# noisystreet/aither

Measured on AMD Instinct MI355X. Metric: Mcell-updates/sec per iteration (residual+LU-SGS), 256^3 block; % HBM roofline, higher is better.
Workload: dtype f64

## Files before the change

### aither_amd/csrc/agx_lusgs.hpp

```cpp
#pragma once
#include "agx_device.hpp"

namespace agx {

enum {
  PA_S = 0,
  PA_B = 3,
  PA_X = 6,
  PA_F = 9,
  PA_COUNT = 15,
  D1_VF = 2 * PA_COUNT,
  D1_AD = D1_VF + 1,
  D2_DOUBLES = 2 * PA_COUNT + 4
};

struct D2Dev {
  double* base;
  long nd2, ps;
  const int* dstart;
  const int* ij_of_pos;
  int Pi, Pj;
  __device__ __forceinline__ double2* pa(int id) const {
    return reinterpret_cast<double2*>(base + 2L * id * nd2);
  }
  __device__ __forceinline__ double* vf() const { return base + (long)D1_VF * nd2; }
  __device__ __forceinline__ double* ad(int d) const { return base + (long)(D1_AD + d) * nd2; }
  __device__ __forceinline__ double ld_ad(int d, long cell) const { return ad(d)[cell]; }
  __device__ __forceinline__ double2 ld_pair(int id, long cell) const { return pa(id)[cell]; }
  __device__ __forceinline__ double ld_vf(long cell) const { return vf()[cell]; }
  __device__ __forceinline__ int jlo(int de) const { return max(0, de - (Pi - 1)); }
  __device__ __forceinline__ int pos2(int ie, int je) const {
    const int de = ie + je;
    return dstart[de] + je - jlo(de);
  }
};

struct KpBlk {
  double* base;
  const int* dstart;
  const agx_bc_surface* surf;
  long nd2, ps;
  int Pi, Pj, ni, nj, nk, ng;
  int nsurf, nsurf_i, nsurf_j, nsurf_k;
  int side_conn[6];
  __device__ __forceinline__ int dstart_cf(int de) const {
    const int a = min(Pi, Pj), bm = max(Pi, Pj);
    if (de <= a) return de * (de + 1) / 2;
    if (de <= bm) return a * (a + 1) / 2 + (de - a) * a;
    const int r = Pi + Pj - 1 - de;
    return Pi * Pj - r * (r + 1) / 2;
  }
  __device__ __forceinline__ const char* pab(int id) const {
    return reinterpret_cast<const char*>(base) + (size_t)id * (size_t)nd2 * 16;
  }
  __device__ __forceinline__ const char* vfb() const {
    return reinterpret_cast<const char*>(base) + (size_t)D1_VF * (size_t)nd2 * 8;
  }
  __device__ __forceinline__ const char* adb(int d) const {
    return reinterpret_cast<const char*>(base) + (size_t)(D1_AD + d) * (size_t)nd2 * 8;
  }
  __device__ __forceinline__ double ld_ad(int d, long cell) const {
    return *reinterpret_cast<const double*>(adb(d) + cell * 8);
  }
  __device__ __forceinline__ double2 ld_pair(int id, long cell) const {
    return *reinterpret_cast<const double2*>(pab(id) + cell * 16);
  }
  __device__ __forceinline__ double ld_vf(long cell) const {
    return *reinterpret_cast<const double*>(vfb() + cell * 8);
  }
  __device__ __forceinline__ int jlo(int de) const { return max(0, de - (Pi - 1)); }
};
struct KpGas { double hf, n, inv_n; };
__device__ __forceinline__ double2 ld16(const char* ubase, unsigned voff) {
  return *reinterpret_cast<const double2*>(ubase + voff);
}
__device__ __forceinline__ double ld8(const char* ubase, unsigned voff) {
  return *reinterpret_cast<const double*>(ubase + voff);
}

}
```

### aither_amd/csrc/agx_lusgs_kernels.hpp

```cpp
#pragma once

namespace agx {

constexpr int TT = 32;
constexpr int TRS = TT + 2;
__device__ __forceinline__ int tile_diag_index(int li, int lj) {
  const int dd = li + lj;
  if (dd < TT) return dd * (dd + 1) / 2 + lj;
  const int r = 2 * TT - 2 - dd;
  return TT * TT - (r + 1) * (r + 2) / 2 + (lj - (dd - (TT - 1)));
}
__device__ __forceinline__ void tile_table(unsigned short* s_tab) {
  const int tid = threadIdx.x;
#pragma unroll
  for (int m = 0; m < 4; ++m) {
    const int li = tid & (TT - 1), lj = (tid >> 5) + 8 * m;
    s_tab[tile_diag_index(li, lj)] = (unsigned short)(li | (lj << 8));
  }
}

__device__ __forceinline__ double kp_tagged(double v, unsigned tag) {
  const unsigned long long u = (unsigned long long)__double_as_longlong(v);
  return __longlong_as_double((long long)((u & ~3ull) | tag));
}
__device__ __forceinline__ bool kp_has_tag(double v, unsigned tag) {
  return ((unsigned)__double_as_longlong(v) & 3u) == tag;
}
__device__ __forceinline__ double cell_visc_factor(const GasDev& g, const double* s) {
  if (!(s[0] > 0.0)) return 0.0;
  return visc_max_term(g, s[0]) * visc_term(g, viscosity(g, temperature(g, s)));
}

__global__ void __launch_bounds__(256) k_d2_geo(BlockDev b) {
  const D2Dev& z = b.d2;
  const long t = (long)blockIdx.x * blockDim.x + threadIdx.x;
  const long n = (long)z.Pi * z.Pj * (b.nk + 2 * b.ng);
  if (t >= n) return;
  const int e3[3] = {(int)(t % z.Pi), (int)((t / z.Pi) % z.Pj), (int)(t / ((long)z.Pi * z.Pj))};
  const long q = b.idx(e3[0] - b.ng, e3[1] - b.ng, e3[2] - b.ng);
  const long p = (long)e3[2] * z.ps + z.pos2(e3[0], e3[1]);
#pragma unroll
  for (int d = 0; d < 3; ++d) {
    double a[4];
#pragma unroll
    for (int c = 0; c < 4; ++c) a[c] = b.fa[d][c][q];
    double ad = 0.0;
    if (e3[d] > 0) {
      const long ql = q - b.stride(d);
      const double v[3] = {b.cen[0][q] - b.cen[0][ql], b.cen[1][q] - b.cen[1][ql],
                           b.cen[2][q] - b.cen[2][ql]};
      const double dist = dot3(v, a);
      ad = dist != 0.0 ? a[3] / dist : 0.0;
    }
    z.pa(PA_F + 2 * d + 0)[p] = make_double2(a[0], a[1]);
    z.pa(PA_F + 2 * d + 1)[p] = make_double2(a[2], a[3]);
    z.ad(d)[p] = ad;
  }
}
__global__ void __launch_bounds__(256) k_d2_x_copy(BlockDev b, int to_d2, unsigned tag) {
  const D2Dev& z = b.d2;
  const long t = (long)blockIdx.x * blockDim.x + threadIdx.x;
  const long n = (long)z.Pi * z.Pj * (b.nk + 2 * b.ng);
  if (t >= n) return;
  const int ie = (int)(t % z.Pi), je = (int)((t / z.Pi) % z.Pj),
            ke = (int)(t / ((long)z.Pi * z.Pj));
  const long q = b.idx(ie - b.ng, je - b.ng, ke - b.ng);
  const long p = (long)ke * z.ps + z.pos2(ie, je);
#pragma unroll
  for (int e = 0; e < AGX_NEQ; ++e) {
    double* xp = reinterpret_cast<double*>(z.pa(PA_X + (e >> 1))) + 2 * p + (e & 1);
    if (to_d2) *xp = kp_tagged(b.x[e][q], tag);
    else b.x[e][q] = *xp;
  }
}

__global__ void __launch_bounds__(256)
k_lusgs_prepare(BlockDev b, GasDev g, SolverDev sp, int write_x, unsigned tag, int again) {
  __shared__ double sv[6][TT][TRS];
  __shared__ unsigned short s_tab[TT * TT];
  const D2Dev& z = b.d2;
  const int tid = threadIdx.x;
  tile_table(s_tab);
  const int i0 = blockIdx.x * TT, j0 = blockIdx.y * TT, ke = blockIdx.z;
  const int k = ke - b.ng;
  const int li = tid & (TT - 1);
  double bb[4][AGX_NEQ], x0[4][AGX_NEQ], ainv[4], vf[4];
#pragma unroll
  for (int m = 0; m < 4; ++m) {
    const int lj = (tid >> 5) + 8 * m;
    const int ie = i0 + li, je = j0 + lj;
    const int i = ie - b.ng, j = je - b.ng;
#pragma unroll
    for (int e = 0; e < AGX_NEQ; ++e) { bb[m][e] = 0.0; x0[m][e] = 0.0; }
    ainv[m] = 1.0;
    vf[m] = 0.0;
    double cs = 0.0;
    if (ie < z.Pi && je < z.Pj) {
      const long q = b.idx(i, j, k);
      double s[AGX_NEQ];
#pragma unroll
      for (int e = 0; e < AGX_NEQ; ++e) { s[e] = b.state[e][q]; sv[e][lj][li] = s[e]; }
      if (s[0] > 0.0) cs = sound_speed(g, s);
      if (sp.viscous) vf[m] = cell_visc_factor(g, s);
      const bool phys = i >= 0 && i < b.ni && j >= 0 && j < b.nj && k >= 0 && k < b.nk;
      if (phys) {
        double dvt = (b.vol[q] * (1.0 + sp.zeta)) / (b.dt[q] * sp.theta);
        if (sp.dual_time_cfl > 0.0) dvt += fmax(b.specrad[q], 0.0) / sp.dual_time_cfl;
        const double a = again ? b.ainv[q] : b.a[q] * sp.relax + dvt;
        b.ainv[q] = a;
        if (sp.diag_add) b.a[q] = a;
        ainv[m] = 1.0 / a;
        rhs_bf(b, g, sp, q, bb[m]);
        if (sp.requires_init) {
#pragma unroll
          for (int e = 0; e < AGX_NEQ; ++e) x0[m][e] = bb[m][e] * ainv[m];
        }
      }
    }
    sv[5][lj][li] = cs;
  }
  __syncthreads();
  long pos[4];
  int tli[4], tlj[4];
#pragma unroll
  for (int m = 0; m < 4; ++m) {
    const unsigned tl = s_tab[tid + 256 * m];
    tli[m] = tl & 0xff; tlj[m] = tl >> 8;
    const int ie = i0 + tli[m], je = j0 + tlj[m];
    pos[m] = -1;
    if (ie < z.Pi && je < z.Pj) {
      pos[m] = (long)ke * z.ps + z.pos2(ie, je);
#pragma unroll
      for (int h = 0; h < 3; ++h)
        z.pa(PA_S + h)[pos[m]] = make_double2(sv[2 * h][tlj[m]][tli[m]], sv[2 * h + 1][tlj[m]][tli[m]]);
    }
  }
  __syncthreads();
#pragma unroll
  for (int m = 0; m < 4; ++m) {
    const int lj = (tid >> 5) + 8 * m;
#pragma unroll
    for (int e = 0; e < AGX_NEQ; ++e) sv[e][lj][li] = bb[m][e];
    sv[5][lj][li] = ainv[m];
  }
  __syncthreads();
  double ai2[4];
#pragma unroll
  for (int m = 0; m < 4; ++m) {
    ai2[m] = sv[5][tlj[m]][tli[m]];
    if (pos[m] >= 0) {
#pragma unroll
      for (int h = 0; h < 3; ++h)
        z.pa(PA_B + h)[pos[m]] = make_double2(sv[2 * h][tlj[m]][tli[m]], sv[2 * h + 1][tlj[m]][tli[m]]);
    }
  }
  __syncthreads();
#pragma unroll
  for (int m = 0; m < 4; ++m) {
    const int lj = (tid >> 5) + 8 * m;
#pragma unroll
    for (int e = 0; e < AGX_NEQ; ++e) sv[e][lj][li] = x0[m][e];
    sv[5][lj][li] = vf[m];
  }
  __syncthreads();
#pragma unroll
  for (int m = 0; m < 4; ++m) {
    if (pos[m] >= 0) {
      if (write_x) {
        z.pa(PA_X + 0)[pos[m]] = make_double2(kp_tagged(sv[0][tlj[m]][tli[m]], tag),
                                              kp_tagged(sv[1][tlj[m]][tli[m]], tag));
        z.pa(PA_X + 1)[pos[m]] = make_double2(kp_tagged(sv[2][tlj[m]][tli[m]], tag),
                                              kp_tagged(sv[3][tlj[m]][tli[m]], tag));
        z.pa(PA_X + 2)[pos[m]] = make_double2(kp_tagged(sv[4][tlj[m]][tli[m]], tag), ai2[m]);
      }
      if (sp.viscous) z.vf()[pos[m]] = sv[5][tlj[m]][tli[m]];
    }
  }
}

struct KpRec {
  double dx[AGX_NEQ];
  double r1, v1[3], p1, h1;
  double r0, v0[3], p0, h0;
  double cs, vf;
};
constexpr int KP_NV = 19;
template <class G>
__device__ __forceinline__ void kp_build_rec(const G& g, const double* s, double cs,
                                             double vf, const double* dx, KpRec& r) {
  const double ke = g.hf + 0.5 * dot3(s + 1, s + 1);
  const double e0 = s[0] * ke + g.n * s[4];
  r.r0 = s[0]; r.p0 = s[4]; r.h0 = e0 + s[4]; r.cs = cs; r.vf = vf;
  const double r1 = s[0] + dx[0];
  const double ir = fast_rcp(r1);
  double v2 = 0.0;
#pragma unroll
  for (int q = 0; q < 3; ++q) {
    r.v0[q] = s[1 + q];
    r.v1[q] = fma(s[0], s[1 + q], dx[1 + q]) * ir;
    v2 = fma(r.v1[q], r.v1[q], v2);
  }
  const double e1 = e0 + dx[4];
  r.r1 = r1;
  r.p1 = (e1 - r1 * (g.hf + 0.5 * v2)) * g.inv_n;
  r.h1 = e1 + r.p1;
#pragma unroll
  for (int e = 0; e < AGX_NEQ; ++e) r.dx[e] = dx[e];
}
__device__ __forceinline__ void kp_term(const KpRec& r, const double* n, double fa, double fad,
                                        bool viscous, bool lower, double* acc) {
  const double vn0 = dot3(r.v0, n), vn1 = dot3(r.v1, n);
  double lam = 0.5 * fa * (fabs(vn0) + r.cs);
  if (viscous) lam = fma(fad, r.vf, lam);
  const double ha = lower ? 0.5 * fa : -0.5 * fa;
  const double m0 = r.r0 * vn0, m1 = r.r1 * vn1, dp = r.p1 - r.p0;
  acc[0] += ha * (m1 - m0) + lam * r.dx[0];
#pragma unroll
  for (int q = 0; q < 3; ++q)
    acc[1 + q] += ha * (fma(m1, r.v1[q], fma(-m0, r.v0[q], dp * n[q]))) + lam * r.dx[1 + q];
  acc[4] += ha * fma(vn1, r.h1, -vn0 * r.h0) + lam * r.dx[4];
}
struct KpFace { double n[3], a, ad; };
template <class Z>
__device__ __forceinline__ void kp_load_face(const Z& z, int d, long p, bool viscous,
                                             KpFace& f) {
  const double2 t0 = z.ld_pair(PA_F + 2 * d, p), t1 = z.ld_pair(PA_F + 2 * d + 1, p);
  f.n[0] = t0.x; f.n[1] = t0.y; f.n[2] = t1.x; f.a = t1.y;
  f.ad = viscous ? z.ld_ad(d, p) : 0.0;
}
template <class Z, class G>
__device__ __forceinline__ void kp_term_mem(const Z& z, const G& g, bool viscous,
                                            long pn, const KpFace& f, bool lower, double* acc) {
  const double2 s0 = z.ld_pair(PA_S, pn), s1 = z.ld_pair(PA_S + 1, pn), s2 = z.ld_pair(PA_S + 2, pn);
  const double2 x0 = z.ld_pair(PA_X, pn), x1 = z.ld_pair(PA_X + 1, pn), x2 = z.ld_pair(PA_X + 2, pn);
  const double s[AGX_NEQ] = {s0.x, s0.y, s1.x, s1.y, s2.x};
  const double dx[AGX_NEQ] = {x0.x, x0.y, x1.x, x1.y, x2.x};
  KpRec r;
  kp_build_rec(g, s, s2.y, viscous ? z.ld_vf(pn) : 0.0, dx, r);
  kp_term(r, f.n, f.a, f.ad, viscous, lower, acc);
}

struct KpArgs {
  int* ticket;
  int* err;
  int spin_limit;
  unsigned tag;
  long long* trace;
};
#ifdef AGX_KP_TRACE
#define KP_STAMP(n) do { if (tid == 0 && kp.trace && k == b.nk / 2) \
    kp.trace[(size_t)(t + 1) * 6 + (n)] = wall_clock64(); } while (0)
#else
#define KP_STAMP(n) do {} while (0)
#endif

struct KpCell {
  double2 o[3];
  double2 s[3], qs[3];
  double vf, qvf;
  KpFace f[3];
  int i, j, pos, use;
  bool act;
};

#ifndef KP_SLEEP
#define KP_SLEEP 2
#endif
template <bool FWD, bool FULL, bool CONN, int CH>
__global__ void __launch_bounds__(256, 1)
k_lusgs_kp(KpBlk b, KpGas g, int viscous, int nsl, KpArgs kp) {
  extern __shared__ double kp_lds[];
  __shared__ int s_kt, s_ok;
  const KpBlk& z = b;
  const int tid = threadIdx.x;
  const int ng = b.ng;
  const int nsteps = b.ni + b.nj - 1;
  const bool visc = viscous != 0;
  if (tid == 0) s_ok = 1;
  for (int n = tid; n < 2 * KP_NV * nsl; n += 256) kp_lds[n] = 0.0;
  for (;;) {
    __syncthreads();
    if (tid == 0) s_kt = atomicAdd(kp.ticket, 1);
    __syncthreads();
    const int kt = __builtin_amdgcn_readfirstlane(s_kt);
    if (kt >= b.nk) break;
    const int k = FWD ? kt : b.nk - 1 - kt;
    const int kq = FWD ? k - 1 : k + 1;
    const bool has_pre = kt > 0;
    const bool k_any = has_pre || (CONN && b.side_conn[FWD ? 4 : 5] != 0);
    const long kbase = (long)(k + ng) * z.ps, qbase = (long)(kq + ng) * z.ps;
    auto step_geom = [&](int t, int& d, int& jmin, int& cnt, int& p0, int& pn) {
      d = FWD ? t : nsteps - 1 - t;
      jmin = max(0, d - (b.ni - 1));
      cnt = min(b.nj - 1, d) - jmin + 1;
      const int de = d + 2 * ng;
      p0 = z.dstart_cf(de) + (jmin + ng) - z.jlo(de);
      const int dq = FWD ? de - 1 : de + 1;
      pn = z.dstart_cf(dq) - z.jlo(dq);
    };
    auto fetch = [&](int t, KpCell* cc) {
      int d, jmin, cnt, p0, pn;
      step_geom(t, d, jmin, cnt, p0, pn);
#pragma unroll
      for (int m = 0; m < CH; ++m) {
        KpCell& c = cc[m];
        const int nraw = tid + 256 * m;
        c.act = nraw < cnt;
        const int n = c.act ? nraw : 0;
        c.j = jmin + n;
        c.i = d - c.j;
        c.pos = p0 + n;
        const unsigned vo = (unsigned)c.pos * 16u;
#pragma unroll
        for (int h = 0; h < 3; ++h) {
          c.o[h] = ld16(z.pab((FWD ? PA_B : PA_X) + h) + kbase * 16, vo);
          c.s[h] = ld16(z.pab(PA_S + h) + kbase * 16, vo);
          c.qs[h] = ld16(z.pab(PA_S + h) + qbase * 16, vo);
        }
        c.vf = ld8(z.vfb() + kbase * 8, (unsigned)c.pos * 8u);
        c.qvf = ld8(z.vfb() + qbase * 8, (unsigned)c.pos * 8u);
        const long fb[3] = {FWD ? kbase : kbase + pn, FWD ? kbase : kbase + pn + 1,
                            FWD ? kbase : kbase + z.ps};
        const unsigned fo[3] = {FWD ? vo : (unsigned)(c.j + ng) * 16u,
                                FWD ? vo : (unsigned)(c.j + ng) * 16u, vo};
#pragma unroll
        for (int q = 0; q < 3; ++q) {
          const double2 t0 = ld16(z.pab(PA_F + 2 * q) + fb[q] * 16, fo[q]);
          const double2 t1 = ld16(z.pab(PA_F + 2 * q + 1) + fb[q] * 16, fo[q]);
          c.f[q].n[0] = t0.x; c.f[q].n[1] = t0.y; c.f[q].n[2] = t1.x; c.f[q].a = t1.y;
          c.f[q].ad = ld8(z.adb(q) + fb[q] * 8, fo[q] >> 1);
        }
        const bool in_i = FWD ? c.i > 0 : c.i < b.ni - 1;
        const bool in_j = FWD ? c.j > 0 : c.j < b.nj - 1;
        int use = (in_i ? 1 : 0) | (in_j ? 2 : 0) | (has_pre ? 4 : 0);
        if (CONN) {
          if (FWD) {
            if (!in_i && bc_is_connection(b, c.i, c.j, k, 1)) use |= 1 | 8;
            if (!in_j && bc_is_connection(b, c.i, c.j, k, 3)) use |= 2 | 16;
            if (!has_pre && bc_is_connection(b, c.i, c.j, k, 5)) use |= 4;
          } else {
            if (!in_i && bc_is_connection(b, c.i + 1, c.j, k, 2)) use |= 1 | 8;
            if (!in_j && bc_is_connection(b, c.i, c.j + 1, k, 4)) use |= 2 | 16;
            if (!has_pre && bc_is_connection(b, c.i, c.j, k + 1, 6)) use |= 4;
          }
        }
        c.use = use;
      }
    };
    KpCell cur[CH], nxt[CH];
    double qx[CH][AGX_NEQ];
    auto qx_request = [&]() {
#pragma unroll
      for (int m = 0; m < CH; ++m) {
#pragma unroll
        for (int e = 0; e < AGX_NEQ; ++e) {
          const double* p = reinterpret_cast<const double*>(
              z.pab(PA_X + (e >> 1)) + qbase * 16 + (unsigned)cur[m].pos * 16u) + (e & 1);
          qx[m][e] = __hip_atomic_load(p, __ATOMIC_RELAXED, __HIP_MEMORY_SCOPE_AGENT);
        }
      }
    };
    auto qx_landed = [&]() {
      unsigned bad = 0;
#pragma unroll
      for (int m = 0; m < CH; ++m) {
#pragma unroll
        for (int e = 0; e < AGX_NEQ; ++e)
          bad |= cur[m].act ? ((unsigned)__double_as_longlong(qx[m][e]) ^ kp.tag) : 0u;
      }
      return (bad & 3u) == 0u;
    };
#pragma unroll
    for (int m = 0; m < CH; ++m) {
      cur[m].act = false;
#pragma unroll
      for (int e = 0; e < AGX_NEQ; ++e) qx[m][e] = 0.0;
    }
    int jmin_prev = 0;
    fetch(0, cur);
    __builtin_amdgcn_s_waitcnt(0x0F70);
    for (int t = 0; t < nsteps; ++t) {
      KP_STAMP(0);
      if (k_any) qx_request();
      fetch(min(t + 1, nsteps - 1), nxt);
      KP_STAMP(1);
      {
        int d, jmin, cnt, p0, pn;
      step_geom(t, d, jmin, cnt, p0, pn);
      double* lw = kp_lds + (size_t)(t & 1) * KP_NV * nsl;
      const double* lr = kp_lds + (size_t)((t & 1) ^ 1) * KP_NV * nsl;
      double accs[CH][AGX_NEQ];
#pragma unroll
      for (int m = 0; m < CH; ++m) {
        const KpCell& c = cur[m];
        double* acc = accs[m];
#pragma unroll
        for (int e = 0; e < AGX_NEQ; ++e) acc[e] = 0.0;
#pragma unroll
        for (int q = 0; q < 2; ++q) {
          const int jn = q == 0 ? c.j : (FWD ? c.j - 1 : c.j + 1);
          const double* rp = lr + min(max(jn - jmin_prev + 1, 0), nsl - 1);
          KpRec r;
#pragma unroll
          for (int e = 0; e < AGX_NEQ; ++e) r.dx[e] = rp[e * nsl];
          r.r1 = rp[5 * nsl]; r.v1[0] = rp[6 * nsl]; r.v1[1] = rp[7 * nsl]; r.v1[2] = rp[8 * nsl];
          r.p1 = rp[9 * nsl]; r.h1 = rp[10 * nsl];
          r.r0 = rp[11 * nsl]; r.v0[0] = rp[12 * nsl]; r.v0[1] = rp[13 * nsl]; r.v0[2] = rp[14 * nsl];
          r.p0 = rp[15 * nsl]; r.h0 = rp[16 * nsl]; r.cs = rp[17 * nsl]; r.vf = rp[18 * nsl];
          if (CONN && (c.use & (8 << q))) {
            const long pg = kbase + pn + (c.j + ng) + (q == 0 ? 0 : (FWD ? -1 : 1));
            kp_term_mem(z, g, visc, pg, c.f[q], FWD, acc);
          } else {
            const bool on = (c.use & (1 << q)) != 0;
            kp_term(r, c.f[q].n, on ? c.f[q].a : 0.0, on ? c.f[q].ad : 0.0, true, FWD, acc);
          }
        }
      }
      KP_STAMP(2);
      if (has_pre) {
        int spins = 0;
        while (!__all(qx_landed())) {
          __builtin_amdgcn_s_sleep(KP_SLEEP);
          if (++spins > kp.spin_limit ||
              ((spins & 63) == 0 &&
               __hip_atomic_load(kp.err, __ATOMIC_RELAXED, __HIP_MEMORY_SCOPE_AGENT) != 0)) {
            s_ok = 0;
            __hip_atomic_store(kp.err, 2, __ATOMIC_RELAXED, __HIP_MEMORY_SCOPE_AGENT);
            break;
          }
          qx_request();
          __builtin_amdgcn_s_waitcnt(0x0F70);
        }
      }
      KP_STAMP(3);
      __builtin_amdgcn_s_waitcnt(0x0F70);
#pragma unroll
      for (int m = 0; m < CH; ++m) {
        const KpCell& c = cur[m];
        double* acc = accs[m];
        const long own = kbase + c.pos;
        if (k_any) {
          const double qs5[AGX_NEQ] = {c.qs[0].x, c.qs[0].y, c.qs[1].x, c.qs[1].y, c.qs[2].x};
          KpRec r;
          kp_build_rec(g, qs5, c.qs[2].y, c.qvf, qx[m], r);
          const bool on = CONN ? (c.use & 4) != 0 : true;
          kp_term(r, c.f[2].n, on ? c.f[2].a : 0.0, on ? c.f[2].ad : 0.0, true, FWD, acc);
        }
        const double ainv = c.o[2].y;
        const double ov[AGX_NEQ] = {c.o[0].x, c.o[0].y, c.o[1].x, c.o[1].y, c.o[2].x};
        double xn[AGX_NEQ];
        if (FULL) {
          const int de = d + 2 * ng;
          const int dqo = FWD ? de + 1 : de - 1;
          const long po = kbase + z.dstart_cf(dqo) - z.jlo(dqo) + (c.j + ng);
          KpFace ff;
          if (FWD) {
            if (c.i < b.ni - 1 || bc_is_connection(b, c.i + 1, c.j, k, 2)) {
              kp_load_face(z, 0, po, visc, ff);
              kp_term_mem(z, g, visc, po, ff, false, acc);
            }
            if (c.j < b.nj - 1 || bc_is_connection(b, c.i, c.j + 1, k, 4)) {
              kp_load_face(z, 1, po + 1, visc, ff);
              kp_term_mem(z, g, visc, po + 1, ff, false, acc);
            }
            if (k < b.nk - 1 || bc_is_connection(b, c.i, c.j, k + 1, 6)) {
              kp_load_face(z, 2, own + z.ps, visc, ff);
              kp_term_mem(z, g, visc, own + z.ps, ff, false, acc);
            }
          } else {
            if (c.i > 0 || bc_is_connection(b, c.i, c.j, k, 1)) {
              kp_load_face(z, 0, own, visc, ff);
              kp_term_mem(z, g, visc, po, ff, true, acc);
            }
            if (c.j > 0 || bc_is_connection(b, c.i, c.j, k, 3)) {
              kp_load_face(z, 1, own, visc, ff);
              kp_term_mem(z, g, visc, po - 1, ff, true, acc);
            }
            if (k > 0 || bc_is_connection(b, c.i, c.j, k, 5)) {
              kp_load_face(z, 2, own, visc, ff);
              kp_term_mem(z, g, visc, own - z.ps, ff, true, acc);
            }
          }
          double bv[AGX_NEQ] = {ov[0], ov[1], ov[2], ov[3], ov[4]};
          if (!FWD) {
            const double2 b0 = z.ld_pair(PA_B, own), b1 = z.ld_pair(PA_B + 1, own),
                          b2 = z.ld_pair(PA_B + 2, own);
            bv[0] = b0.x; bv[1] = b0.y; bv[2] = b1.x; bv[3] = b1.y; bv[4] = b2.x;
          }
#pragma unroll
          for (int e = 0; e < AGX_NEQ; ++e) xn[e] = (bv[e] + acc[e]) * ainv;
        } else if (FWD) {
#pragma unroll
          for (int e = 0; e < AGX_NEQ; ++e) xn[e] = (ov[e] + acc[e]) * ainv;
        } else {
#pragma unroll
          for (int e = 0; e < AGX_NEQ; ++e) xn[e] = ov[e] + acc[e] * ainv;
        }
#pragma unroll
        for (int e = 0; e < AGX_NEQ; ++e) xn[e] = kp_tagged(xn[e], kp.tag);
        if (c.act) {
          typedef double v2d __attribute__((ext_vector_type(2)));
          const unsigned po = (unsigned)c.pos * 16u;
          const v2d v0 = {xn[0], xn[1]}, v1 = {xn[2], xn[3]}, v2 = {xn[4], ainv};
          asm volatile("s_nop 4\n\tglobal_store_dwordx4 %0, %1, %2 sc1\n\ts_nop 1"
                       :: "v"(po), "v"(v0), "s"(z.pab(PA_X + 0) + kbase * 16) : "memory");
          asm volatile("s_nop 4\n\tglobal_store_dwordx4 %0, %1, %2 sc1\n\ts_nop 1"
                       :: "v"(po), "v"(v1), "s"(z.pab(PA_X + 1) + kbase * 16) : "memory");
          asm volatile("s_nop 4\n\tglobal_store_dwordx4 %0, %1, %2 sc1\n\ts_nop 1"
                       :: "v"(po), "v"(v2), "s"(z.pab(PA_X + 2) + kbase * 16) : "memory");
        }
        const double s5[AGX_NEQ] = {c.s[0].x, c.s[0].y, c.s[1].x, c.s[1].y, c.s[2].x};
        KpRec r;
        kp_build_rec(g, s5, c.s[2].y, c.vf, xn, r);
        if (c.act) {
        double* wp = lw + (c.j - jmin + 1);
#pragma unroll
        for (int e = 0; e < AGX_NEQ; ++e) wp[e * nsl] = xn[e];
        wp[5 * nsl] = r.r1; wp[6 * nsl] = r.v1[0]; wp[7 * nsl] = r.v1[1]; wp[8 * nsl] = r.v1[2];
        wp[9 * nsl] = r.p1; wp[10 * nsl] = r.h1;
        wp[11 * nsl] = r.r0; wp[12 * nsl] = r.v0[0]; wp[13 * nsl] = r.v0[1]; wp[14 * nsl] = r.v0[2];
        wp[15 * nsl] = r.p0; wp[16 * nsl] = r.h0; wp[17 * nsl] = r.cs; wp[18 * nsl] = r.vf;
        }
      }
      jmin_prev = jmin;
      }
      KP_STAMP(4);
      __syncthreads();
      if (!s_ok) return;
#pragma unroll
      for (int m = 0; m < CH; ++m) cur[m] = nxt[m];
      KP_STAMP(5);
    }
  }
}

__global__ void __launch_bounds__(256)
k_matrix_resid_d2(BlockDev b, GasDev g, SolverDev sp, int nsplit, NormPartial* partials) {
  const D2Dev& z = b.d2;
  const int nchunk = (z.Pi * z.Pj + 255) / 256;
  const int per = (nchunk + 8 * nsplit - 1) / (8 * nsplit);
  const int xcd = blockIdx.x % 8, m = blockIdx.x / 8;
  const int band = (m / (per * b.nk)) * 8 + xcd, rem = m % (per * b.nk);
  const int k = rem / per, chunk = band * per + rem % per;
  const int t = chunk * 256 + threadIdx.x;
  const bool visc = sp.viscous != 0;
  double r[AGX_NEQ] = {0, 0, 0, 0, 0};
  bool active = false;
  if (chunk < nchunk && t < z.Pi * z.Pj) {
    const int ij = z.ij_of_pos[t];
    const int ie = ij & 0xffff, je = ij >> 16;
    const int i = ie - b.ng, j = je - b.ng;
    active = i >= 0 && i < b.ni && j >= 0 && j < b.nj;
    if (active) {
      const long kbase = (long)(k + b.ng) * z.ps;
      const long own = kbase + t;
      const int de = ie + je;
      const long plo = kbase + z.dstart[de - 1] - z.jlo(de - 1) + je;
      const long pup = kbase + z.dstart[de + 1] - z.jlo(de + 1) + je;
      double acc[AGX_NEQ] = {0, 0, 0, 0, 0};
      const long nlo[3] = {plo, plo - 1, own - z.ps}, nup[3] = {pup, pup + 1, own + z.ps};
      const int c3[3] = {i, j, k}, n3[3] = {b.ni, b.nj, b.nk};
      KpFace ff;
#pragma unroll
      for (int d = 0; d < 3; ++d) {
        if (c3[d] > 0 || bc_is_connection(b, i, j, k, 2 * d + 1)) {
          kp_load_face(z, d, own, visc, ff);
          kp_term_mem(z, g, visc, nlo[d], ff, true, acc);
        }
      }
#pragma unroll
      for (int d = 0; d < 3; ++d) {
        if (c3[d] < n3[d] - 1 ||
            bc_is_connection(b, i + (d == 0), j + (d == 1), k + (d == 2), 2 * d + 2)) {
          kp_load_face(z, d, nup[d], visc, ff);
          kp_term_mem(z, g, visc, nup[d], ff, false, acc);
        }
      }
      const double2 x0 = z.pa(PA_X)[own], x1 = z.pa(PA_X + 1)[own], x2 = z.pa(PA_X + 2)[own];
      const double2 b0 = z.pa(PA_B)[own], b1 = z.pa(PA_B + 1)[own], b2 = z.pa(PA_B + 2)[own];
      const double a = 1.0 / b2.y;
      const double xv[AGX_NEQ] = {x0.x, x0.y, x1.x, x1.y, x2.x};
      const double bv[AGX_NEQ] = {b0.x, b0.y, b1.x, b1.y, b2.x};
#pragma unroll
      for (int e = 0; e < AGX_NEQ; ++e) r[e] = -(xv[e] * a - acc[e] - bv[e]);
    }
  }
  norm_block_reduce(r, 0, active, partials + blockIdx.x);
}

#ifndef AGX_MR_WAVES
#define AGX_MR_WAVES 1
#endif
__global__ void __launch_bounds__(256, AGX_MR_WAVES)
k_matrix_resid_d2m(BlockDev b, GasDev g, SolverDev sp, int kc, NormPartial* partials) {
  const D2Dev& z = b.d2;
  const int nchunk = (z.Pi * z.Pj + 255) / 256;
  const int per = (nchunk + 7) / 8;
  const int xcd = blockIdx.x % 8, m = blockIdx.x / 8;
  const int chunk = xcd * per + m % per, kch = m / per;
  const int k0 = kch * kc, k1 = min(k0 + kc, b.nk);
  const int t = chunk * 256 + threadIdx.x;
  const bool visc = sp.viscous != 0;
  double l2[AGX_NEQ] = {0, 0, 0, 0, 0};
  bool active = false;
  int i = 0, j = 0, je = 0, de = 0;
  if (chunk < nchunk && t < z.Pi * z.Pj) {
    const int ij = z.ij_of_pos[t];
    const int ie = ij & 0xffff;
    je = ij >> 16;
    i = ie - b.ng; j = je - b.ng; de = ie + je;
    active = i >= 0 && i < b.ni && j >= 0 && j < b.nj;
  }
  if (active) {
    const long qlo = z.dstart[de - 1] - z.jlo(de - 1) + je;
    const long qup = z.dstart[de + 1] - z.jlo(de + 1) + je;
    struct Col { double s[AGX_NEQ], cs, x[AGX_NEQ], vf; };
    auto ld_col = [&](long p, Col& c) {
      const double2 s0 = z.ld_pair(PA_S, p), s1 = z.ld_pair(PA_S + 1, p), s2 = z.ld_pair(PA_S + 2, p);
      const double2 x0 = z.ld_pair(PA_X, p), x1 = z.ld_pair(PA_X + 1, p), x2 = z.ld_pair(PA_X + 2, p);
      c.s[0] = s0.x; c.s[1] = s0.y; c.s[2] = s1.x; c.s[3] = s1.y; c.s[4] = s2.x; c.cs = s2.y;
      c.x[0] = x0.x; c.x[1] = x0.y; c.x[2] = x1.x; c.x[3] = x1.y; c.x[4] = x2.x;
      c.vf = visc ? z.ld_vf(p) : 0.0;
    };
    auto col_term = [&](const Col& c, const KpFace& f, bool lower, double* acc) {
      KpRec r;
      kp_build_rec(g, c.s, c.cs, c.vf, c.x, r);
      kp_term(r, f.n, f.a, f.ad, visc, lower, acc);
    };
    Col cm, c0, cp;
    KpFace fk0, fk1;
    long own = (long)(k0 + b.ng) * z.ps + t;
    ld_col(own - z.ps, cm);
    ld_col(own, c0);
    kp_load_face(z, 2, own, visc, fk0);
    for (int k = k0; k < k1; ++k, own += z.ps) {
      const long kbase = own - t;
      ld_col(own + z.ps, cp);
      kp_load_face(z, 2, own + z.ps, visc, fk1);
      const double2 b0 = z.pa(PA_B)[own], b1 = z.pa(PA_B + 1)[own], b2 = z.pa(PA_B + 2)[own];
      double acc[AGX_NEQ] = {0, 0, 0, 0, 0};
      KpFace ff;
      if (i > 0 || bc_is_connection(b, i, j, k, 1)) {
        kp_load_face(z, 0, own, visc, ff);
        kp_term_mem(z, g, visc, kbase + qlo, ff, true, acc);
      }
      if (j > 0 || bc_is_connection(b, i, j, k, 3)) {
        kp_load_face(z, 1, own, visc, ff);
        kp_term_mem(z, g, visc, kbase + qlo - 1, ff, true, acc);
      }
      if (k > 0 || bc_is_connection(b, i, j, k, 5)) col_term(cm, fk0, true, acc);
      if (i < b.ni - 1 || bc_is_connection(b, i + 1, j, k, 2)) {
        kp_load_face(z, 0, kbase + qup, visc, ff);
        kp_term_mem(z, g, visc, kbase + qup, ff, false, acc);
      }
      if (j < b.nj - 1 || bc_is_connection(b, i, j + 1, k, 4)) {
        kp_load_face(z, 1, kbase + qup + 1, visc, ff);
        kp_term_mem(z, g, visc, kbase + qup + 1, ff, false, acc);
      }
      if (k < b.nk - 1 || bc_is_connection(b, i, j, k + 1, 6)) col_term(cp, fk1, false, acc);
      const double a = 1.0 / b2.y;
      const double bv[AGX_NEQ] = {b0.x, b0.y, b1.x, b1.y, b2.x};
#pragma unroll
      for (int e = 0; e < AGX_NEQ; ++e) {
        const double r = -(c0.x[e] * a - acc[e] - bv[e]);
        l2[e] += r * r;
      }
      cm = c0; c0 = cp; fk0 = fk1;
    }
  }
  norm_block_fold(l2, -1.0e300, 0x7fffffffffffffffLL, partials + blockIdx.x);
}

__global__ void __launch_bounds__(256)
k_update_d2(BlockDev b, GasDev g, SolverDev sp, int last_mm, NormPartial* partials) {
  __shared__ double sv[AGX_NEQ][TT][TRS];
  __shared__ unsigned short s_tab[TT * TT];
  const D2Dev& z = b.d2;
  const int tid = threadIdx.x;
  tile_table(s_tab);
  __syncthreads();
  const int i0 = blockIdx.x * TT, j0 = blockIdx.y * TT, k = blockIdx.z;
#pragma unroll
  for (int m = 0; m < 4; ++m) {
    const unsigned tl = s_tab[tid + 256 * m];
    const int tli = tl & 0xff, tlj = tl >> 8;
    const int i = i0 + tli, j = j0 + tlj;
    if (i < b.ni && j < b.nj) {
      const long p = (long)(k + b.ng) * z.ps + z.pos2(i + b.ng, j + b.ng);
      const double2 x0 = z.pa(PA_X)[p], x1 = z.pa(PA_X + 1)[p], x2 = z.pa(PA_X + 2)[p];
      sv[0][tlj][tli] = x0.x; sv[1][tlj][tli] = x0.y; sv[2][tlj][tli] = x1.x;
      sv[3][tlj][tli] = x1.y; sv[4][tlj][tli] = x2.x;
    }
  }
  __syncthreads();
  const int li = tid & (TT - 1);
  double l2[AGX_NEQ] = {0, 0, 0, 0, 0};
  double vmax = -1.0e300;
  long long vlin = 0x7fffffffffffffffLL;
#pragma unroll
  for (int m = 0; m < 4; ++m) {
    const int lj = (tid >> 5) + 8 * m;
    const int i = i0 + li, j = j0 + lj;
    if (i < b.ni && j < b.nj) {
      const long q = b.idx(i, j, k);
      double r[AGX_NEQ], s[AGX_NEQ], du[AGX_NEQ], ns[AGX_NEQ];
      load5(b.resid, q, r);
      load5(b.state, q, s);
#pragma unroll
      for (int e = 0; e < AGX_NEQ; ++e) du[e] = sv[e][lj][li];
      update_prim_with_cons(g, s, du, ns);
      store5(b.state, q, ns);
      if (sp.bdf2 && last_mm) {
        double u[AGX_NEQ];
        load5(b.consn, q, u);
        store5(b.consnm1, q, u);
      }
      const long lin0 = (((long)k * b.nj + j) * b.ni + i) * AGX_NEQ;
#pragma unroll
      for (int e = 0; e < AGX_NEQ; ++e) {
        l2[e] += r[e] * r[e];
        if (r[e] > vmax || (r[e] == vmax && lin0 + e < vlin)) { vmax = r[e]; vlin = lin0 + e; }
      }
    }
  }
  const long bid = ((long)blockIdx.z * gridDim.y + blockIdx.y) * gridDim.x + blockIdx.x;
  norm_block_fold(l2, vmax, vlin, partials + bid);
}

}
```

Baseline: 1496.

## Precompute per-plane base pointers, incrementally advance diagonal geometry, ping-pong cells, AoS LDS

```diff
diff --git a/aither_amd/csrc/agx_kp_geom.hpp b/aither_amd/csrc/agx_kp_geom.hpp
--- /dev/null
+++ b/aither_amd/csrc/agx_kp_geom.hpp
@@ -0,0 +1,71 @@
+#pragma once
+
+#if defined(__HIPCC__)
+#define AGX_KG_HD __host__ __device__ __forceinline__
+#else
+#define AGX_KG_HD inline
+#endif
+
+namespace agx {
+
+AGX_KG_HD int kg_min(int a, int b) { return a < b ? a : b; }
+AGX_KG_HD int kg_max(int a, int b) { return a > b ? a : b; }
+
+struct KpPlane {
+  int Pi, Pj;
+  AGX_KG_HD int jlo(int de) const { return kg_max(0, de - (Pi - 1)); }
+  AGX_KG_HD int len(int de) const { return kg_min(de, Pj - 1) - jlo(de) + 1; }
+  AGX_KG_HD int dstart_cf(int de) const {
+    const int a = kg_min(Pi, Pj), bm = kg_max(Pi, Pj);
+    if (de <= a) return de * (de + 1) / 2;
+    if (de <= bm) return a * (a + 1) / 2 + (de - a) * a;
+    const int r = Pi + Pj - 1 - de;
+    return Pi * Pj - r * (r + 1) / 2;
+  }
+};
+
+struct KpGeom {
+  int d, jmin, cnt;
+  int de, ds;
+  int pb, pbs;
+};
+
+template <bool FWD>
+AGX_KG_HD KpGeom kp_geom_first(const KpPlane& z, int ni, int nj, int ng) {
+  KpGeom g;
+  g.d = FWD ? 0 : ni + nj - 2;
+  g.jmin = kg_max(0, g.d - (ni - 1));
+  g.cnt = kg_min(nj - 1, g.d) - g.jmin + 1;
+  g.de = g.d + 2 * ng;
+  g.ds = z.dstart_cf(g.de);
+  g.pb = g.ds - z.jlo(g.de);
+  const int dq = FWD ? g.de - 1 : g.de + 1;
+  g.pbs = z.dstart_cf(dq) - z.jlo(dq);
+  return g;
+}
+template <bool FWD>
+AGX_KG_HD KpGeom kp_geom_next(const KpPlane& z, int ni, int nj, const KpGeom& g) {
+  KpGeom n;
+  n.d = FWD ? g.d + 1 : g.d - 1;
+  n.jmin = kg_max(0, n.d - (ni - 1));
+  n.cnt = kg_min(nj - 1, n.d) - n.jmin + 1;
+  n.de = FWD ? g.de + 1 : g.de - 1;
+  n.ds = FWD ? g.ds + z.len(g.de) : g.ds - z.len(n.de);
+  n.pb = n.ds - z.jlo(n.de);
+  n.pbs = g.pb;
+  return n;
+}
+
+AGX_KG_HD KpGeom kp_geom_pick(bool first, const KpGeom& a, const KpGeom& b) {
+  KpGeom g;
+  g.d = first ? a.d : b.d;
+  g.jmin = first ? a.jmin : b.jmin;
+  g.cnt = first ? a.cnt : b.cnt;
+  g.de = first ? a.de : b.de;
+  g.ds = first ? a.ds : b.ds;
+  g.pb = first ? a.pb : b.pb;
+  g.pbs = first ? a.pbs : b.pbs;
+  return g;
+}
+
+}
diff --git a/aither_amd/csrc/agx_lusgs.hpp b/aither_amd/csrc/agx_lusgs.hpp
--- a/aither_amd/csrc/agx_lusgs.hpp
+++ b/aither_amd/csrc/agx_lusgs.hpp
@@ -1,5 +1,6 @@
 #pragma once
 #include "agx_device.hpp"
+#include "agx_kp_geom.hpp"
 
 namespace agx {
 
@@ -43,13 +44,7 @@
   int Pi, Pj, ni, nj, nk, ng;
   int nsurf, nsurf_i, nsurf_j, nsurf_k;
   int side_conn[6];
-  __device__ __forceinline__ int dstart_cf(int de) const {
-    const int a = min(Pi, Pj), bm = max(Pi, Pj);
-    if (de <= a) return de * (de + 1) / 2;
-    if (de <= bm) return a * (a + 1) / 2 + (de - a) * a;
-    const int r = Pi + Pj - 1 - de;
-    return Pi * Pj - r * (r + 1) / 2;
-  }
+  __device__ __forceinline__ KpPlane plane() const { return KpPlane{Pi, Pj}; }
   __device__ __forceinline__ const char* pab(int id) const {
     return reinterpret_cast<const char*>(base) + (size_t)id * (size_t)nd2 * 16;
   }
@@ -68,14 +63,13 @@
   __device__ __forceinline__ double ld_vf(long cell) const {
     return *reinterpret_cast<const double*>(vfb() + cell * 8);
   }
-  __device__ __forceinline__ int jlo(int de) const { return max(0, de - (Pi - 1)); }
 };
 struct KpGas { double hf, n, inv_n; };
-__device__ __forceinline__ double2 ld16(const char* ubase, unsigned voff) {
-  return *reinterpret_cast<const double2*>(ubase + voff);
+__device__ __forceinline__ double2 ld16(const char* ubase, unsigned voff, int imm = 0) {
+  return *reinterpret_cast<const double2*>(ubase + voff + imm);
 }
-__device__ __forceinline__ double ld8(const char* ubase, unsigned voff) {
-  return *reinterpret_cast<const double*>(ubase + voff);
+__device__ __forceinline__ double ld8(const char* ubase, unsigned voff, int imm = 0) {
+  return *reinterpret_cast<const double*>(ubase + voff + imm);
 }
 
 }
diff --git a/aither_amd/csrc/agx_lusgs_kernels.hpp b/aither_amd/csrc/agx_lusgs_kernels.hpp
--- a/aither_amd/csrc/agx_lusgs_kernels.hpp
+++ b/aither_amd/csrc/agx_lusgs_kernels.hpp
@@ -189,7 +189,7 @@
 __device__ __forceinline__ void kp_build_rec(const G& g, const double* s, double cs,
                                              double vf, const double* dx, KpRec& r) {
   const double ke = g.hf + 0.5 * dot3(s + 1, s + 1);
-  const double e0 = s[0] * ke + g.n * s[4];
+  const double e0 = fma(g.n, s[4], s[0] * ke);
   r.r0 = s[0]; r.p0 = s[4]; r.h0 = e0 + s[4]; r.cs = cs; r.vf = vf;
   const double r1 = s[0] + dx[0];
   const double ir = fast_rcp(r1);
@@ -260,6 +260,7 @@
   double vf, qvf;
   KpFace f[3];
   int i, j, pos, use;
+  unsigned vk, vq;
   bool act;
 };
 
@@ -287,48 +288,57 @@
     const int k = FWD ? kt : b.nk - 1 - kt;
     const int kq = FWD ? k - 1 : k + 1;
     const bool has_pre = kt > 0;
-    const bool k_any = has_pre || (CONN && b.side_conn[FWD ? 4 : 5] != 0);
+    const bool k_any = __builtin_amdgcn_readfirstlane(
+                           (int)(has_pre || (CONN && b.side_conn[FWD ? 4 : 5] != 0))) != 0;
     const long kbase = (long)(k + ng) * z.ps, qbase = (long)(kq + ng) * z.ps;
-    auto step_geom = [&](int t, int& d, int& jmin, int& cnt, int& p0, int& pn) {
-      d = FWD ? t : nsteps - 1 - t;
-      jmin = max(0, d - (b.ni - 1));
-      cnt = min(b.nj - 1, d) - jmin + 1;
-      const int de = d + 2 * ng;
-      p0 = z.dstart_cf(de) + (jmin + ng) - z.jlo(de);
-      const int dq = FWD ? de - 1 : de + 1;
-      pn = z.dstart_cf(dq) - z.jlo(dq);
-    };
-    auto fetch = [&](int t, KpCell* cc) {
-      int d, jmin, cnt, p0, pn;
-      step_geom(t, d, jmin, cnt, p0, pn);
+    const long lob = FWD ? qbase : kbase;
+    const unsigned ps16 = (unsigned)z.ps * 16u;
+    const unsigned offk = FWD ? ps16 : 0u, offq = FWD ? 0u : ps16;
+    const char* const bS[3] = {z.pab(PA_S) + lob * 16, z.pab(PA_S + 1) + lob * 16,
+                               z.pab(PA_S + 2) + lob * 16};
+    const char* const bX[3] = {z.pab(PA_X) + lob * 16, z.pab(PA_X + 1) + lob * 16,
+                               z.pab(PA_X + 2) + lob * 16};
+    const char* const bO[3] = {FWD ? z.pab(PA_B) + lob * 16 : bX[0],
+                               FWD ? z.pab(PA_B + 1) + lob * 16 : bX[1],
+                               FWD ? z.pab(PA_B + 2) + lob * 16 : bX[2]};
+    const char* const bF[6] = {z.pab(PA_F) + lob * 16, z.pab(PA_F + 1) + lob * 16,
+                               z.pab(PA_F + 2) + lob * 16, z.pab(PA_F + 3) + lob * 16,
+                               z.pab(PA_F + 4) + lob * 16, z.pab(PA_F + 5) + lob * 16};
+    const char* const bAD[3] = {z.adb(0) + lob * 8, z.adb(1) + lob * 8, z.adb(2) + lob * 8};
+    const char* const bVF = z.vfb() + lob * 8;
+    const KpPlane pl = z.plane();
+    auto fetch = [&](const KpGeom& gm, KpCell* cc) __attribute__((always_inline)) {
+      const int p0 = gm.pb + gm.jmin + ng;
+      const unsigned gk = (unsigned)p0 * 16u + offk, gq = (unsigned)p0 * 16u + offq;
+      const unsigned gf = (unsigned)(gm.pbs + gm.jmin + ng) * 16u;
 #pragma unroll
       for (int m = 0; m < CH; ++m) {
         KpCell& c = cc[m];
         const int nraw = tid + 256 * m;
-        c.act = nraw < cnt;
+        c.act = nraw < gm.cnt;
         const int n = c.act ? nraw : 0;
-        c.j = jmin + n;
-        c.i = d - c.j;
+        c.j = gm.jmin + n;
+        c.i = gm.d - c.j;
         c.pos = p0 + n;
-        const unsigned vo = (unsigned)c.pos * 16u;
+        const unsigned ln = (unsigned)n * 16u;
+        c.vk = gk + ln;
+        c.vq = gq + ln;
 #pragma unroll
         for (int h = 0; h < 3; ++h) {
-          c.o[h] = ld16(z.pab((FWD ? PA_B : PA_X) + h) + kbase * 16, vo);
-          c.s[h] = ld16(z.pab(PA_S + h) + kbase * 16, vo);
-          c.qs[h] = ld16(z.pab(PA_S + h) + qbase * 16, vo);
-        }
-        c.vf = ld8(z.vfb() + kbase * 8, (unsigned)c.pos * 8u);
-        c.qvf = ld8(z.vfb() + qbase * 8, (unsigned)c.pos * 8u);
-        const long fb[3] = {FWD ? kbase : kbase + pn, FWD ? kbase : kbase + pn + 1,
-                            FWD ? kbase : kbase + z.ps};
-        const unsigned fo[3] = {FWD ? vo : (unsigned)(c.j + ng) * 16u,
-                                FWD ? vo : (unsigned)(c.j + ng) * 16u, vo};
+          c.o[h] = ld16(bO[h], c.vk);
+          c.s[h] = ld16(bS[h], c.vk);
+          c.qs[h] = ld16(bS[h], c.vq);
+        }
+        c.vf = ld8(bVF, c.vk >> 1);
+        c.qvf = ld8(bVF, c.vq >> 1);
+        const unsigned fo[3] = {FWD ? c.vk : gf + ln, FWD ? c.vk : gf + ln, FWD ? c.vk : c.vq};
+        const int fi[3] = {0, FWD ? 0 : 16, 0};
 #pragma unroll
         for (int q = 0; q < 3; ++q) {
-          const double2 t0 = ld16(z.pab(PA_F + 2 * q) + fb[q] * 16, fo[q]);
-          const double2 t1 = ld16(z.pab(PA_F + 2 * q + 1) + fb[q] * 16, fo[q]);
+          const double2 t0 = ld16(bF[2 * q], fo[q], fi[q]);
+          const double2 t1 = ld16(bF[2 * q + 1], fo[q], fi[q]);
           c.f[q].n[0] = t0.x; c.f[q].n[1] = t0.y; c.f[q].n[2] = t1.x; c.f[q].a = t1.y;
-          c.f[q].ad = ld8(z.adb(q) + fb[q] * 8, fo[q] >> 1);
+          c.f[q].ad = ld8(bAD[q], fo[q] >> 1, fi[q] >> 1);
         }
         const bool in_i = FWD ? c.i > 0 : c.i < b.ni - 1;
         const bool in_j = FWD ? c.j > 0 : c.j < b.nj - 1;
@@ -347,20 +357,19 @@
         c.use = use;
       }
     };
-    KpCell cur[CH], nxt[CH];
+    KpCell ca[CH], cb[CH];
     double qx[CH][AGX_NEQ];
-    auto qx_request = [&]() {
+    auto qx_request = [&](const KpCell* cur) __attribute__((always_inline)) {
 #pragma unroll
       for (int m = 0; m < CH; ++m) {
 #pragma unroll
         for (int e = 0; e < AGX_NEQ; ++e) {
-          const double* p = reinterpret_cast<const double*>(
-              z.pab(PA_X + (e >> 1)) + qbase * 16 + (unsigned)cur[m].pos * 16u) + (e & 1);
+          const double* p = reinterpret_cast<const double*>(bX[e >> 1] + cur[m].vq + (e & 1) * 8);
           qx[m][e] = __hip_atomic_load(p, __ATOMIC_RELAXED, __HIP_MEMORY_SCOPE_AGENT);
         }
       }
     };
-    auto qx_landed = [&]() {
+    auto qx_landed = [&](const KpCell* cur) __attribute__((always_inline)) {
       unsigned bad = 0;
 #pragma unroll
       for (int m = 0; m < CH; ++m) {
@@ -372,23 +381,26 @@
     };
 #pragma unroll
     for (int m = 0; m < CH; ++m) {
-      cur[m].act = false;
 #pragma unroll
       for (int e = 0; e < AGX_NEQ; ++e) qx[m][e] = 0.0;
     }
     int jmin_prev = 0;
-    fetch(0, cur);
+    KpGeom ga = kp_geom_first<FWD>(pl, b.ni, b.nj, ng), gb = ga;
+    fetch(ga, ca);
     __builtin_amdgcn_s_waitcnt(0x0F70);
-    for (int t = 0; t < nsteps; ++t) {
+    auto step = [&](auto par, const int t, const KpCell* cur, const KpGeom& gm, KpCell* nxt,
+                    KpGeom& gn) __attribute__((always_inline)) -> bool {
+      constexpr int PAR = decltype(par)::value;
       KP_STAMP(0);
-      if (k_any) qx_request();
-      fetch(min(t + 1, nsteps - 1), nxt);
+      if (k_any) qx_request(cur);
+      const KpGeom adv = kp_geom_next<FWD>(pl, b.ni, b.nj, gm);
+      gn = kp_geom_pick(t + 1 < nsteps, adv, gm);
+      fetch(gn, nxt);
       KP_STAMP(1);
       {
-        int d, jmin, cnt, p0, pn;
-      step_geom(t, d, jmin, cnt, p0, pn);
-      double* lw = kp_lds + (size_t)(t & 1) * KP_NV * nsl;
-      const double* lr = kp_lds + (size_t)((t & 1) ^ 1) * KP_NV * nsl;
+      const int jmin = gm.jmin, pn = gm.pbs;
+      double* lw = kp_lds + (size_t)PAR * KP_NV * nsl;
+      const double* lr = kp_lds + (size_t)(PAR ^ 1) * KP_NV * nsl;
       double accs[CH][AGX_NEQ];
 #pragma unroll
       for (int m = 0; m < CH; ++m) {
@@ -399,14 +411,14 @@
 #pragma unroll
         for (int q = 0; q < 2; ++q) {
           const int jn = q == 0 ? c.j : (FWD ? c.j - 1 : c.j + 1);
-          const double* rp = lr + min(max(jn - jmin_prev + 1, 0), nsl - 1);
+          const double* rp = lr + min(max(jn - jmin_prev + 1, 0), nsl - 1) * KP_NV;
           KpRec r;
 #pragma unroll
-          for (int e = 0; e < AGX_NEQ; ++e) r.dx[e] = rp[e * nsl];
-          r.r1 = rp[5 * nsl]; r.v1[0] = rp[6 * nsl]; r.v1[1] = rp[7 * nsl]; r.v1[2] = rp[8 * nsl];
-          r.p1 = rp[9 * nsl]; r.h1 = rp[10 * nsl];
-          r.r0 = rp[11 * nsl]; r.v0[0] = rp[12 * nsl]; r.v0[1] = rp[13 * nsl]; r.v0[2] = rp[14 * nsl];
-          r.p0 = rp[15 * nsl]; r.h0 = rp[16 * nsl]; r.cs = rp[17 * nsl]; r.vf = rp[18 * nsl];
+          for (int e = 0; e < AGX_NEQ; ++e) r.dx[e] = rp[e];
+          r.r1 = rp[5]; r.v1[0] = rp[6]; r.v1[1] = rp[7]; r.v1[2] = rp[8];
+          r.p1 = rp[9]; r.h1 = rp[10];
+          r.r0 = rp[11]; r.v0[0] = rp[12]; r.v0[1] = rp[13]; r.v0[2] = rp[14];
+          r.p0 = rp[15]; r.h0 = rp[16]; r.cs = rp[17]; r.vf = rp[18];
           if (CONN && (c.use & (8 << q))) {
             const long pg = kbase + pn + (c.j + ng) + (q == 0 ? 0 : (FWD ? -1 : 1));
             kp_term_mem(z, g, visc, pg, c.f[q], FWD, acc);
@@ -419,7 +431,7 @@
       KP_STAMP(2);
       if (has_pre) {
         int spins = 0;
-        while (!__all(qx_landed())) {
+        while (!__all(qx_landed(cur))) {
           __builtin_amdgcn_s_sleep(KP_SLEEP);
           if (++spins > kp.spin_limit ||
               ((spins & 63) == 0 &&
@@ -428,7 +440,7 @@
             __hip_atomic_store(kp.err, 2, __ATOMIC_RELAXED, __HIP_MEMORY_SCOPE_AGENT);
             break;
           }
-          qx_request();
+          qx_request(cur);
           __builtin_amdgcn_s_waitcnt(0x0F70);
         }
       }
@@ -450,9 +462,7 @@
         const double ov[AGX_NEQ] = {c.o[0].x, c.o[0].y, c.o[1].x, c.o[1].y, c.o[2].x};
         double xn[AGX_NEQ];
         if (FULL) {
-          const int de = d + 2 * ng;
-          const int dqo = FWD ? de + 1 : de - 1;
-          const long po = kbase + z.dstart_cf(dqo) - z.jlo(dqo) + (c.j + ng);
+          const long po = kbase + adv.pb + (c.j + ng);
           KpFace ff;
           if (FWD) {
             if (c.i < b.ni - 1 || bc_is_connection(b, c.i + 1, c.j, k, 2)) {
@@ -500,36 +510,41 @@
         for (int e = 0; e < AGX_NEQ; ++e) xn[e] = kp_tagged(xn[e], kp.tag);
         if (c.act) {
           typedef double v2d __attribute__((ext_vector_type(2)));
-          const unsigned po = (unsigned)c.pos * 16u;
+          const unsigned po = c.vk;
           const v2d v0 = {xn[0], xn[1]}, v1 = {xn[2], xn[3]}, v2 = {xn[4], ainv};
           asm volatile("s_nop 4\n\tglobal_store_dwordx4 %0, %1, %2 sc1\n\ts_nop 1"
-                       :: "v"(po), "v"(v0), "s"(z.pab(PA_X + 0) + kbase * 16) : "memory");
+                       :: "v"(po), "v"(v0), "s"(bX[0]) : "memory");
           asm volatile("s_nop 4\n\tglobal_store_dwordx4 %0, %1, %2 sc1\n\ts_nop 1"
-                       :: "v"(po), "v"(v1), "s"(z.pab(PA_X + 1) + kbase * 16) : "memory");
+                       :: "v"(po), "v"(v1), "s"(bX[1]) : "memory");
           asm volatile("s_nop 4\n\tglobal_store_dwordx4 %0, %1, %2 sc1\n\ts_nop 1"
-                       :: "v"(po), "v"(v2), "s"(z.pab(PA_X + 2) + kbase * 16) : "memory");
+                       :: "v"(po), "v"(v2), "s"(bX[2]) : "memory");
         }
         const double s5[AGX_NEQ] = {c.s[0].x, c.s[0].y, c.s[1].x, c.s[1].y, c.s[2].x};
         KpRec r;
         kp_build_rec(g, s5, c.s[2].y, c.vf, xn, r);
         if (c.act) {
-        double* wp = lw + (c.j - jmin + 1);
-#pragma unroll
-        for (int e = 0; e < AGX_NEQ; ++e) wp[e * nsl] = xn[e];
-        wp[5 * nsl] = r.r1; wp[6 * nsl] = r.v1[0]; wp[7 * nsl] = r.v1[1]; wp[8 * nsl] = r.v1[2];
-        wp[9 * nsl] = r.p1; wp[10 * nsl] = r.h1;
-        wp[11 * nsl] = r.r0; wp[12 * nsl] = r.v0[0]; wp[13 * nsl] = r.v0[1]; wp[14 * nsl] = r.v0[2];
-        wp[15 * nsl] = r.p0; wp[16 * nsl] = r.h0; wp[17 * nsl] = r.cs; wp[18 * nsl] = r.vf;
+        double* wp = lw + (c.j - jmin + 1) * KP_NV;
+#pragma unroll
+        for (int e = 0; e < AGX_NEQ; ++e) wp[e] = xn[e];
+        wp[5] = r.r1; wp[6] = r.v1[0]; wp[7] = r.v1[1]; wp[8] = r.v1[2];
+        wp[9] = r.p1; wp[10] = r.h1;
+        wp[11] = r.r0; wp[12] = r.v0[0]; wp[13] = r.v0[1]; wp[14] = r.v0[2];
+        wp[15] = r.p0; wp[16] = r.h0; wp[17] = r.cs; wp[18] = r.vf;
         }
       }
       jmin_prev = jmin;
       }
       KP_STAMP(4);
       __syncthreads();
-      if (!s_ok) return;
-#pragma unroll
-      for (int m = 0; m < CH; ++m) cur[m] = nxt[m];
+      const bool ok = __builtin_amdgcn_readfirstlane(s_ok) != 0;
       KP_STAMP(5);
+      return ok;
+    };
+    for (int t = 0;;) {
+      if (!step(std::integral_constant<int, 0>{}, t, ca, ga, cb, gb)) return;
+      if (++t >= nsteps) break;
+      if (!step(std::integral_constant<int, 1>{}, t, cb, gb, ca, ga)) return;
+      if (++t >= nsteps) break;
     }
   }
 }
```

New measurement: 1509, median of 6. Within noise of the previous version (+0.9%).
